# Michaelszeng/GCS-ADMM

Measured on AMD Instinct MI355X. Metric: admm_iterations_per_sec, higher is better.
Workload: dtype f64; 1 GPU; benchmark4; V=42, E=94, n=2, state_dtype=f64, state_columns=incidence, inner_arithmetic=f64, vertex_program=workgroup, vertex_solves=warm start from the previous iteration's record (csrc/warm_start.h), parallelism=1 GPU

## Files before the change

### gcs_admm_amd/csrc/vertex_wg.h

```cpp
#pragma once
#include <type_traits>

#include "gcs_math.h"
#include "step_args.h"
#include "warm_start.h"

#if defined(__HIP_DEVICE_COMPILE__)
#define WG_DEVICE 1
#else
#define WG_DEVICE 0
#endif

namespace gcs_wg {

using gcs_math::REG_DELTA;
using gcs_math::rcp;
using gcs_math::rcp1;
using gcs_math::rsqrt_nr;
using gcs_math::sqrt_nr;

#ifndef GCS_WG_THREADS
#define GCS_WG_THREADS 256
#endif
constexpr int WG_THREADS = GCS_WG_THREADS;
// ... 15 lines not shown
__device__ __forceinline__ int wg_tid()
{
    int t = (int)threadIdx.x;
    asm volatile("" : "+v"(t));
    return t;
}
#define WG_FOR(i, cnt) for (int i = gcs_wg::wg_tid(), i##_end = (cnt); i < i##_end; i += gcs_wg::WG_THREADS)
#define WG_FOR_AT(i, cnt, start) for (int i = (gcs_wg::wg_tid() - (start)) & (gcs_wg::WG_THREADS - 1), i##_end = (cnt); i < i##_end; i += gcs_wg::WG_THREADS)
#define WG_SYNC() gcs_wg::wg_barrier<WG_VM>()
#define WG_ONE() if (gcs_wg::wg_tid() == 0)
#define WG_CONE() if (gcs_wg::wg_tid() == gcs_wg::WG_THREADS - 1)
#define WG_CONE2(l) for (int l = gcs_wg::wg_tid() - (gcs_wg::WG_THREADS - 2); l >= 0 && l < 2; l = 2)
#define WG_WAVE0() if (gcs_wg::wg_tid() < 64)
#define WG_FIRST_WAVES(w, cnt) for (int w = gcs_wg::wg_tid() >> 6; w < (cnt); w += gcs_wg::WG_WAVES)
#define WG_ITEM_FOR(q, i, count, PER)                                                                                          \
    for (int t_ = gcs_wg::wg_tid(), w_ = t_ >> 6, l_ = t_ & 63,                                                                \
             n_ = w_ < gcs_wg::WG_ITEM_WAVES ? (((count) - w_ + gcs_wg::WG_ITEM_WAVES - 1) / gcs_wg::WG_ITEM_WAVES) * (PER) : 0;  \
         l_ < n_; l_ += 64)                                                                                                    \
        if (const int qq_ = l_ / (PER), i = l_ - qq_ * (PER), q = w_ + gcs_wg::WG_ITEM_WAVES * qq_; true)
#define WG_REPL_FOR(i, cnt) for (int i = (gcs_wg::wg_tid() >> 6) < gcs_wg::WG_ITEM_WAVES ? (gcs_wg::wg_tid() & 63) : (cnt), i##_end = (cnt); i < i##_end; i += 64)
#define WG_WAVE_SYNC() gcs_wg::wg_wave_sync<WG_VM>()
#define WG_FENCE() asm volatile("" ::: "memory")
#else
#define WG_FENCE() do { } while (0)
#ifdef GCS_WG_REVERSE
#define WG_FOR(i, cnt) for (int i = (cnt) - 1; i >= 0; --i)
#else
#define WG_FOR(i, cnt) for (int i = 0, i##_end = (cnt); i < i##_end; ++i)
#endif
#define WG_FOR_AT(i, cnt, start) WG_FOR(i, ((void)(start), (cnt)))
#define WG_SYNC() do { } while (0)
#define WG_ONE() if (true)
#define WG_CONE() if (true)
#define WG_CONE2(l) for (int l = 0; l < 2; ++l)
#define WG_WAVE0() if (true)
#define WG_FIRST_WAVES(w, cnt) for (int w = 0; w < (cnt); ++w)
#define WG_ITEM_FOR(q, i, count, PER) WG_FOR(t_, (count) * (PER)) if (const int q = t_ / (PER), i = t_ - q * (PER); true)
#define WG_REPL_FOR(i, cnt) WG_FOR(i, cnt)
#define WG_WAVE_SYNC() do { } while (0)
#endif

#if defined(GCS_WG_TIMING) && defined(__HIPCC__)
__device__ unsigned long long g_wg_cycles[64];
__device__ unsigned long long g_wg_counts[64];
__device__ unsigned long long g_wg_wave_cycles[64 * 8];
#endif
#if defined(GCS_WG_TIMING) && WG_DEVICE
__device__ __forceinline__ void wg_stamp(int id, unsigned long long &last)
{
    if (blockIdx.x == 0) {
        const unsigned long long t = __builtin_amdgcn_s_memtime();
        if (threadIdx.x == 0) {
            atomicAdd(&g_wg_cycles[id], t - last);
            atomicAdd(&g_wg_counts[id], 1ull);
        }
        last = t;
    }
}
__device__ __forceinline__ void wg_arrive(int id, unsigned long long last)
{
    if (blockIdx.x == 0) {
        const unsigned long long t = __builtin_amdgcn_s_memtime();
        if ((threadIdx.x & 63) == 0) atomicAdd(&g_wg_wave_cycles[id * 8 + ((threadIdx.x >> 6) & 7)], t - last);
    }
}
#define WG_ARRIVE(id) gcs_wg::wg_arrive(id, wg_last_stamp)
#define WG_STAMP(id) gcs_wg::wg_stamp(id, wg_last_stamp)
#define WG_STAMP_INIT() unsigned long long wg_last_stamp = __builtin_amdgcn_s_memtime()
#else
#define WG_STAMP(id) do { } while (0)
#define WG_ARRIVE(id) do { } while (0)
#define WG_STAMP_INIT() do { } while (0)
#endif

struct Place {
    int off = 0;
    GCS_HD int at(int cnt)
    {
        const int start = off & (WG_THREADS - 1);
        off = (off + cnt + 63) & ~63;
        return start;
    }
};

template <int N> struct WD {
    static constexpr int NW = 2 * N + 1, NX = 2 * N, NB1 = 4 * N + 1, Q = N + 1, NS = N * (N + 1) / 2;
    static constexpr int TA = 2 * NS + 2 * N + 1;
};

constexpr int pad2(int x) { return (x + 1) & ~1; }
template <int N> struct WSoc {
    static constexpr int Q = N + 1;
    static constexpr int SS = 0, LS = Q, WB = 2 * Q, LT = 3 * Q, CV = LT + Q, SU = CV + N, DSSA = SU + N * N, DLSA = DSSA + Q,
                         DSS = DLSA + Q, DLS = DSS + Q, KS = DLS + Q, SIZE = KS + Q;
};
enum { SC_T = 0, SC_DT, SC_DTA, SC_ALPHA, SC_CONEFAIL, SC_C0, SC_ETA, SC_GT, SC_AMAXC, SC_C1C, SC_C2C, SC_AMAXC2, SC_N = 12 };
template <int N> struct WL {
    using D = WD<N>;
    static constexpr int NW = D::NW, NX = D::NX, NB1 = D::NB1;
    static constexpr int CEN = 0, XV = CEN + pad2(N), DX = XV + pad2(NX), NU = DX + pad2(NX), DNU = NU + pad2(2 * NW),
                         BS = DNU + pad2(2 * NW), BSI = BS + pad2(2 * NW * NW), BXS = BSI + pad2(2 * NW * NW),
                         PIVS = BXS + pad2(2 * NW * NX), BG = PIVS + pad2(2 * NW), XBG = BG + pad2(2 * NW), XBX = XBG + pad2(2 * NX),
                         XS = XBX + pad2(2 * NX * NX), RP = XS + pad2(NX * N), VV = RP + pad2(2 * NW), WW = VV + pad2(2 * NW), M = WW + pad2(2 * NW),
                         PIVM = M + pad2(NB1 * NB1), RHS = PIVM + pad2(NB1), SOL = RHS + pad2(NB1),
                         SOC = SOL + pad2(NB1), PQ = SOC + pad2(WSoc<N>::SIZE), PC = PQ + pad2(NX + NW), SC = PC + pad2(NX + NW), RED = SC + pad2(SC_N), FIXED = RED + 3 * 3 * WG_WAVES;
    static constexpr int P = 0, DW = P + pad2(NW), TG = DW + pad2(NW), TF = TG + pad2(NW), LB = TF + pad2(N), KB = LB + 2, DLB = KB + 2,
                         PIV = DLB + 2, G0 = PIV + pad2(NW), GU = G0 + pad2(NW), GX = GU + pad2(NW), TE = GX + pad2(NX),
                         RV = TE + pad2(NW), K = RV + pad2(NW), X = K + pad2(NW * NW), B = X + pad2(NW * NX), ROWS = B + pad2(NW * NW);
    static GCS_HD int unit_stride(int m) { return (ROWS + 12 * m) | 1; }
    static GCS_HD int total(int U, int m) { return FIXED + pad2(U * unit_stride(m)) + pad2(m * N) + pad2(m); }
    static GCS_HD int units_doubles(int U, int m) { return pad2(U * unit_stride(m)); }
};
template <int N> struct WLBox {
    using G = WL<N>;
    using D = WD<N>;
    static constexpr int NW = D::NW, NX = D::NX, NB1 = D::NB1;
    static constexpr int CEN = G::CEN, XV = G::XV, DX = G::DX, NU = G::NU, DNU = G::DNU, BS = G::BS, BSI = G::BSI, BXS = G::BXS, PIVS = G::PIVS,
                         BG = G::BG, XBG = G::XBG, XBX = G::XBX, XS = G::XS, RP = G::RP, VV = G::VV, WW = G::WW, M = G::M, PIVM = G::PIVM,
                         RHS = G::RHS, SOL = G::SOL, SOC = G::SOC, PQ = G::PQ, PC = G::PC, SC = G::SC, RED = G::RED, FIXED = G::FIXED;
    static constexpr int P = G::P, DW = G::DW, TG = G::TG, TF = G::TF, LB = G::LB, KB = G::KB, DLB = G::DLB, G0 = G::G0, GU = G::GU, GX = G::GX,
                         TE = G::TE, RV = G::RV;
    static constexpr int KD = G::K, KY = KD + pad2(NX), KYY = KY + pad2(NX), XD = KYY + 2, XY = XD + pad2(NX),
                         BD = XY + pad2(NX), BW = BD + pad2(NX), BRS = BW + pad2(NW), BQ = BRS + 2, ROWS = BQ + pad2(NX);
    static GCS_HD int unit_stride(int m) { return (ROWS + 12 * m) | 1; }
    static GCS_HD int total(int U, int m) { return FIXED + pad2(U * unit_stride(m)) + pad2(m * N) + pad2(m); }
    static GCS_HD int units_doubles(int U, int m) { return pad2(U * unit_stride(m)); }
};
template <int N> GCS_HD int wg_lds_doubles(int U, int m, bool box = false) { return box ? WLBox<N>::total(U, m) : WL<N>::total(U, m); }
constexpr int WG_MAX_N = 8;
inline bool wg_has_box(int n) { return n == 3 || n == 6; }
inline int wg_lds_doubles_n(int n, int U, int m, bool box = false)
{
    box = box && wg_has_box(n);
    switch (n) {
    case 1: return wg_lds_doubles<1>(U, m);
    case 2: return wg_lds_doubles<2>(U, m);
    case 3: return wg_lds_doubles<3>(U, m, box);
    case 4: return wg_lds_doubles<4>(U, m);
    case 5: return wg_lds_doubles<5>(U, m);
    case 6: return wg_lds_doubles<6>(U, m, box);
    case 7: return wg_lds_doubles<7>(U, m);
    default: return wg_lds_doubles<8>(U, m);
    }
}

struct alignas(8) WgF2 { float a, b; };

template <class T> struct WgArgs : gcsadmm_k::StepArgs<T> {
    int n_vtx;
    const int *vtx;
    const double *prox_q = nullptr, *prox_c = nullptr;
    const int *order = nullptr;
    int *unit_iters = nullptr;
};

struct Red3 { double mn, s1, s2; };

#if WG_DEVICE
template <int SH> __device__ __forceinline__ double dpp_row_shr(double x, double ident)
{
    const int ilo = __double2loint(ident), ihi = __double2hiint(ident);
    const int lo = __builtin_amdgcn_update_dpp(ilo, __double2loint(x), 0x110 + SH, 0xf, 0xf, false);
    const int hi = __builtin_amdgcn_update_dpp(ihi, __double2hiint(x), 0x110 + SH, 0xf, 0xf, false);
    return __hiloint2double(hi, lo);
}
__device__ __forceinline__ double lane_bcast(double x, int lane)
// ... 142 lines not shown
#pragma unroll
        for (int k = i + 1; k < DIM; ++k) s -= Lm[k * DIM + i] * x[k];
        x[i] = s;
        if constexpr (LOWREG) out[i * ldo + c] = s;
        if constexpr (DIM > 9) WG_FENCE();
    }
    if constexpr (!LOWREG) {
#pragma unroll
        for (int i = 0; i < DIM; ++i) out[i * ldo + c] = x[i];
    }
}

template <int Q> GCS_HD void soc_apply_W(const double *wb, double eta, const double *x, double *y)
{
    double dd = 0;
#pragma unroll
    for (int k = 1; k < Q; ++k) dd += wb[k] * x[k];
    const double f = x[0] + dd * rcp(1.0 + wb[0]);
    y[0] = eta * (wb[0] * x[0] + dd);
#pragma unroll
    for (int k = 1; k < Q; ++k) y[k] = eta * (x[k] + wb[k] * f);
}
template <int Q> GCS_HD void soc_apply_Wi(const double *wb, double eta, const double *x, double *y)
{
    double dd = 0;
#pragma unroll
    for (int k = 1; k < Q; ++k) dd += wb[k] * x[k];
    const double ieta = rcp(eta), f = -x[0] + dd * rcp(1.0 + wb[0]);
    y[0] = ieta * (wb[0] * x[0] - dd);
#pragma unroll
    for (int k = 1; k < Q; ++k) y[k] = ieta * (x[k] + wb[k] * f);
}
template <int Q> GCS_HD void soc_apply_W2(const double *wb, double eta, const double *x, double *y)
{
    double vx = wb[0] * x[0];
#pragma unroll
    for (int k = 1; k < Q; ++k) vx -= wb[k] * x[k];
    const double ieta = rcp(eta), ie2 = ieta * ieta;
    y[0] = ie2 * (2.0 * wb[0] * vx - x[0]);
#pragma unroll
    for (int k = 1; k < Q; ++k) y[k] = ie2 * (x[k] - 2.0 * wb[k] * vx);
}

#define WG_ROWS_BEGIN_(pl, DS)                                                                                                 \
    WG_FOR_AT(rt_, (BOX ? U * 2 * N : U * m2), (pl).at(BOX ? U * 2 * N : U * m2)) {                                            \
        int u, i, jk_;                                                                                                         \
        if constexpr (BOX) { u = rt_ / (2 * N); const int ik_ = rt_ - u * (2 * N); i = ik_ / N; jk_ = ik_ - i * N; }           \
        else { u = fdiv(rt_, inv_m2); const int rem_ = rt_ - u * m2; i = rem_ >= m; jk_ = rem_ - i * m; }                      \
        double *un = UN(u);                                                                                                    \
        double ap_ = 0, ax_ = 0, adp_ = 0, adx_ = 0;                                                                           \
        if constexpr (BOX) {                                                                                                   \
            ap_ = un[W::P + i * N + jk_]; ax_ = sm[W::XV + i * N + jk_];                                                       \
            if (DS) { adp_ = un[W::DW + i * N + jk_]; adx_ = sm[W::DX + i * N + jk_]; }                                        \
        } else {                                                                                                               \
            _Pragma("unroll") for (int k_ = 0; k_ < N; ++k_) {                                                                 \
                const double a_ = A[jk_ * N + k_];                                                                             \
                ap_ += a_ * un[W::P + i * N + k_]; ax_ += a_ * sm[W::XV + i * N + k_];                                         \
                if (DS) { adp_ += a_ * un[W::DW + i * N + k_]; adx_ += a_ * sm[W::DX + i * N + k_]; }                          \
            }                                                                                                                  \
        }                                                                                                                      \
        const double yy_ = un[W::P + 2 * N], dy_ = DS ? un[W::DW + 2 * N] : 0.0;                                               \
        _Pragma("unroll") for (int rq_ = 0; rq_ < (BOX ? 4 : 2); ++rq_) {                                                      \
            const int ty = BOX ? rq_ >> 1 : rq_, j = BOX ? jk_ + (rq_ & 1) * N : jk_, ro = ty * m2 + i * m + j;                \
            const double sg_ = (BOX && (rq_ & 1)) ? -1.0 : 1.0, b_ = BC[j];                                                    \
            const double s = ty == 0 ? b_ * yy_ - sg_ * ap_ : b_ * (1.0 - yy_) - sg_ * (ax_ - ap_);                            \
            const double ds = ty == 0 ? b_ * dy_ - sg_ * adp_ : -(b_ * dy_) - sg_ * (adx_ - adp_);                             \
            (void)ds;
#define WG_ROWS_BEGIN(pl) WG_ROWS_BEGIN_(pl, false)
#define WG_ROWS_BEGIN_DS(pl) WG_ROWS_BEGIN_(pl, true)
#define WG_ROWS_END() }}

template <int N, class T, bool BOX = false, bool SPLIT = false>
GCS_HD void wg_solve_vertex(const WgArgs<T> &a, int v, double rho, double mu_scale, double *sm, int &status_out, int &iters_out,
                            double *units = nullptr)
{
    using D = WD<N>;
    using SO = WSoc<N>;
    using W = std::conditional_t<BOX, WLBox<N>, WL<N>>;
    constexpr int NW = D::NW, NX = D::NX, NB1 = D::NB1, Q = D::Q, NS = D::NS, TA = D::TA;
#ifndef GCS_WG_CONE_PAIR_MAXN
#define GCS_WG_CONE_PAIR_MAXN 3
#endif
    constexpr bool CONE_PAIR = N <= GCS_WG_CONE_PAIR_MAXN;
    const bool prox = a.prox_q != nullptr;
    const int lo = a.inc_ptr[v], d = prox ? 0 : a.inc_ptr[v + 1] - lo, d_in = prox ? 0 : a.deg_in[v], d_out = d - d_in;
    const bool sides = d > 0;
    const int p0 = a.poly_ptr[v], m = a.poly_ptr[v + 1] - p0;
    const int U = d + 1, R = 4 * m, m2 = 2 * m;
    const int US = W::unit_stride(m);
    const float inv_m2 = 1.0f / (float)m2;
    double *const UB = SPLIT ? units : sm + W::FIXED;
    auto UN = [&](int u) -> double * { return UB + u * US; };
    constexpr bool WG_VM = SPLIT;
    const int oLAM = W::ROWS, oR1 = W::ROWS + R, oR2 = W::ROWS + 2 * R;
    double *const PA = sm + W::FIXED + (SPLIT ? 0 : pad2(U * US));
    const double *A = PA, *BC = PA + pad2(m * N), *CEN = sm + W::CEN;
    double *SOC = sm + W::SOC, *SC = sm + W::SC;
    int red_phase = 0;
    WG_STAMP_INIT();
    const int deg = (4 * m + 2) * (d + 1) + 1;
    const double inv_deg = 1.0 / (double)deg;
    auto side_of = [&](int u) { return (u - 1) >= d_in ? 1 : 0; };
    auto side_lo = [&](int s) { return s ? d_in + 1 : 1; };
    auto side_hi = [&](int s) { return s ? d : d_in; };

    using WR = gcs_ws::WRec<N>;
    double *const wrec = (a.warm != nullptr && !prox) ? a.warm + a.warm_ptr[v] : nullptr;
    const int WUS = WR::unit_stride(m);
    double dtm = 0.0;
    Place pl0;
    WG_FOR_AT(t, d * NW, pl0.at(d * NW)) {
        const int e = t / NW, w = t - e * NW, edge = a.inc_edge[lo + e];
        const bool out = e >= d_in;
        const int inc = gcsadmm_k::state_column(a, lo, e, edge, out);
        double *un = UN(e + 1);
        const double Tw = gcsadmm_k::consensus_target(a, w, edge, inc, mu_scale);
        int slot = -1;
        if (w == 2 * N) slot = 2 * N;
        else if (out) slot = w;
        else if (w < N) { un[W::TF + w] = Tw; un[W::TG + N + w] = 0.0; }
        else slot = w - N;
        if (slot >= 0) {
            un[W::TG + slot] = Tw;
            if (wrec) dtm = fmax(dtm, fabs(Tw - wrec[WR::UNITS + (e + 1) * WUS + WR::TG + slot]));
        }
    }
    WG_FOR_AT(t, m * N, pl0.at(m * N)) PA[t] = a.poly_A[(size_t)p0 * N + t];
    WG_FOR_AT(j, m + N, pl0.at(m + N)) {
        if (j < m) PA[pad2(m * N) + j] = a.poly_bc[p0 + j];
        else sm[W::CEN + (j - m)] = a.center[(size_t)v * N + (j - m)];
    }
    if (prox) {
        WG_FOR(k, NX + NW) {
            sm[W::PQ + k] = a.prox_q[(size_t)v * (NX + NW) + k];
            sm[W::PC + k] = a.prox_c[(size_t)v * (NX + NW) + k];
        }
    }
    bool use_warm = false;
    double mu_ref = gcs_ws::WS_COLD_REF, ws_dT = -1.0;
    if (wrec) {
        const Red3 rt = wg_reduce<WG_VM>(Red3{-dtm, 0.0, 0.0}, sm + W::RED, red_phase);
        const bool comparable = wg_uniform((int)(wrec[0] == 1.0 && wrec[1] == rho)) != 0;
        ws_dT = wg_uniform(comparable ? -rt.mn * rho : -1.0);
        use_warm = wg_uniform((int)(comparable && ws_dT <= gcs_ws::ws_theta(wrec))) != 0;
        if (use_warm) mu_ref = wg_uniform(fmax(gcs_ws::WS_MU_MIN, gcs_ws::WS_KAPPA * ws_dT));
    }
    const bool ws_started_warm = use_warm;
    const float inv_R2 = 1.0f / (float)(R / 2);

    WG_STAMP(0);
    auto gval = [&](const double *un, int u, int k, bool wk) {
        double g = un[W::G0 + k];
        if (wk) {
            g += un[W::GU + k];
            if (u == 0 && k < 2 * N) g += k < N ? -SOC[SO::KS + 1 + k] : SOC[SO::KS + 1 + (k - N)];
        }
        return g;
    };
    auto te_tasks = [&](Place &pl, bool wk) {
        WG_FOR_AT(t, d * NW, pl.at(d * NW)) {
            const int u = 1 + t / NW, i = t - (u - 1) * NW;
            double *un = UN(u);
            double s = 0;
            if constexpr (BOX) {
                double wg = 0;
#pragma unroll
                for (int k = 0; k < NW; ++k) wg += un[W::BW + k] * gval(un, u, k, wk);
                s = -(un[W::BRS] * un[W::BW + i]) * wg;
                if (i < 2 * N) s -= un[W::BD + i] * gval(un, u, i, wk);
            } else {
#pragma unroll
                for (int k = 0; k < NW; ++k) s -= un[W::B + i * NW + k] * gval(un, u, k, wk);
            }
            un[W::TE + i] = s;
        }
    };
    auto bg_tasks = [&](Place &pl) {
        WG_FOR_AT(t, 2 * NW, pl.at(2 * NW)) {
            const int s = t / NW, i = t - s * NW;
            double acc = 0;
#pragma unroll 4
            for (int u = side_lo(s); u <= side_hi(s); ++u) acc += UN(u)[W::TE + i];
            sm[W::BG + t] = acc;
        }
        WG_FOR_AT(t, 2 * NX, pl.at(2 * NX)) {
            const int part = t / NX, c = t - part * NX, h = c / N;
            const int ulo = part ? 1 + d / 2 : 1, uhi = part ? d : d / 2;
            double acc = 0;
#pragma unroll 2
            for (int u = ulo; u <= uhi; ++u) {
                const double *un = UN(u);
                if constexpr (BOX) acc += un[W::XD + c] * un[W::TE + c] + un[W::XY + c] * un[W::TE + 2 * N];
                else {
#pragma unroll
                    for (int k = 0; k < N; ++k) acc += un[W::X + (h * N + k) * NX + c] * un[W::TE + h * N + k];
                    acc += un[W::X + 2 * N * NX + c] * un[W::TE + 2 * N];
                }
            }
            sm[W::XBG + t] = acc;
        }
    };
    auto v_tasks = [&](Place &pl) {
        WG_FOR_AT(t, 2 * NW, pl.at(2 * NW)) {
            const int s = t / NW, i = t - s * NW;
            const double *Bsi = sm + W::BSI + s * NW * NW;
            double acc = 0;
#pragma unroll
            for (int k = 0; k < NW; ++k) acc += Bsi[i * NW + k] * (sm[W::RP + s * NW + k] - sm[W::BG + s * NW + k]);
            sm[W::VV + t] = acc;
        }
    };
    auto rhs_tasks = [&](Place &pl, bool wk) {
        const double *u0 = UN(0);
        auto base_z = [&](int i) { return -gval(u0, 0, i, wk) - sm[W::VV + i] - sm[W::VV + NW + i]; };
        WG_FOR_AT(q, NX, pl.at(NX)) {
            double r = -REG_DELTA * sm[W::XV + q] - sm[W::XBG + q] - sm[W::XBG + NX + q];
            if (prox) r -= sm[W::PQ + q] * (sm[W::XV + q] + CEN[q < N ? q : q - N] - sm[W::PC + q]);
            if (wk) r -= sm[W::SOL + q];
            for (int s = 0; s < 2; ++s) {
                const double *BXs = sm + W::BXS + s * NW * NX;
#pragma unroll
                for (int i = 0; i < NW; ++i) r -= BXs[i * NX + q] * sm[W::VV + s * NW + i];
            }
            sm[W::RHS + q] = r;
        }
        WG_FOR_AT(k, N, pl.at(N))
            sm[W::RHS + NX + k] = base_z(k) + SOC[SO::CV + k] * SC[SC_GT] * rcp(SC[SC_C0]);
        WG_FOR_AT(k, N, pl.at(N))
            sm[W::RHS + NX + N + k] = base_z(k) + base_z(N + k);
        WG_FOR_AT(k, 1, pl.at(1)) sm[W::RHS + NX + 2 * N + k] = base_z(2 * N);
    };
    auto solve_head = [&](bool wk) {
        {
            Place pl;
            te_tasks(pl, wk);
            if (wk) {
                WG_FOR_AT(q, NX, pl.at(NX)) {
                    double acc = 0;
#pragma unroll 4
                    for (int u = 0; u <= d; ++u) acc += UN(u)[W::GX + q];
                    sm[W::SOL + q] = acc;
                }
            }
        }
        WG_ARRIVE(30);
        WG_SYNC();
        WG_STAMP(30);
        { Place pl; bg_tasks(pl); }
        WG_ARRIVE(31);
        WG_SYNC();
        WG_STAMP(31);
        { Place pl; v_tasks(pl); }
        WG_ARRIVE(32);
        WG_SYNC();
        WG_STAMP(32);
        { Place pl; rhs_tasks(pl, wk); }
        WG_ARRIVE(33);
        WG_SYNC();
        WG_STAMP(33);
    };
    auto cone_dir = [&](int dt_slot, bool wk, double (&xs)[Q], double (&dl)[Q]) {
        const double *u0 = UN(0);
        double wb[Q], ys[Q];
        xs[0] = SC[dt_slot];
#pragma unroll
        for (int k = 0; k < N; ++k) xs[1 + k] = u0[W::DW + k] - u0[W::DW + N + k];
#pragma unroll
        for (int k = 0; k < Q; ++k) wb[k] = SOC[SO::WB + k];
        soc_apply_W2<Q>(wb, SC[SC_ETA], xs, ys);
#pragma unroll
        for (int k = 0; k < Q; ++k) dl[k] = (wk ? SOC[SO::KS + k] : 0.0) - SOC[SO::LS + k] - ys[k];
    };
    auto solve_tail = [&](int dt_slot, bool wk) {
        WG_WAVE0() wave_ldl_solve<NB1>(sm + W::M, sm + W::PIVM, sm + W::RHS, sm + W::SOL);
        WG_ARRIVE(34);
        WG_SYNC();
        WG_STAMP(34);
        auto dzeta = [&](int i) { return i < N ? sm[W::SOL + NX + i] + sm[W::SOL + NX + N + i] : sm[W::SOL + NX + i]; };
        Place plw;
        WG_FOR_AT(t, 2 * NW, plw.at(2 * NW)) {
            const int s = t / NW, i = t - s * NW;
            const double *BXs = sm + W::BXS + s * NW * NX;
            double acc = dzeta(i) + (sm[W::RP + t] - sm[W::BG + t]);
#pragma unroll
            for (int c = 0; c < NX; ++c) acc += BXs[i * NX + c] * sm[W::SOL + c];
            sm[W::WW + t] = acc;
        }
        WG_FOR_AT(t, NX + NW + 1, plw.at(NX + NW + 1)) {
            if (t < NX) sm[W::DX + t] = sm[W::SOL + t];
            else if (t < NX + NW) UN(0)[W::DW + (t - NX)] = dzeta(t - NX);
            else {
                double acc = -SC[SC_GT];
#pragma unroll
                for (int k = 0; k < N; ++k) acc -= SOC[SO::CV + k] * sm[W::SOL + NX + k];
                SC[dt_slot] = acc * rcp(SC[SC_C0]);
            }
        }
        WG_ARRIVE(36);
        WG_SYNC();
        WG_STAMP(36);
        auto cone_bounds = [&](int l) {
            const int oDS = wk ? SO::DSS : SO::DSSA, oDL = wk ? SO::DLS : SO::DLSA;
            double xs[Q], dl[Q], bs[Q], dr[Q];
            cone_dir(dt_slot, wk, xs, dl);
            double c1c = 0, c2c = 0;
#pragma unroll
            for (int k = 0; k < Q; ++k) {
                const double sk = SOC[SO::SS + k], lk = SOC[SO::LS + k];
                SOC[oDS + k] = xs[k]; SOC[oDL + k] = dl[k];
                c1c += sk * dl[k] + lk * xs[k];
                c2c += xs[k] * dl[k];
                bs[k] = l == 1 ? lk : sk; dr[k] = l == 1 ? dl[k] : xs[k];
            }
            SC[SC_C1C] = c1c; SC[SC_C2C] = c2c;
            SC[l == 1 ? SC_AMAXC2 : SC_AMAXC] = gcs_math::soc_max_step<Q>(bs, dr);
            if (l == 2) SC[SC_AMAXC2] = gcs_math::soc_max_step<Q>(SOC + SO::LS, dl);
        };
        if constexpr (CONE_PAIR) { WG_CONE2(l) cone_bounds(l); }
        else { WG_CONE() cone_bounds(2); }
        WG_REPL_FOR(t, 2 * NW) {
            const int s = t / NW, i = t - s * NW;
            const double *Bsi = sm + W::BSI + s * NW * NW;
            double acc = 0;
#pragma unroll
            for (int k = 0; k < NW; ++k) acc += Bsi[i * NW + k] * sm[W::WW + s * NW + k];
            sm[W::DNU + t] = acc;
        }
        WG_WAVE_SYNC();
        WG_ITEM_FOR(q, i, d, NW) {
            const int u = 1 + q;
            double *un = UN(u);
            double acc = -gval(un, u, i, wk) + sm[W::DNU + side_of(u) * NW + i];
            if constexpr (BOX) {
                if (i < 2 * N) acc -= un[W::XD + i] * sm[W::DX + i];
                else {
#pragma unroll
                    for (int c = 0; c < NX; ++c) acc -= un[W::XY + c] * sm[W::DX + c];
                }
            } else if (i < 2 * N) {
                const int h = i / N;
#pragma unroll
                for (int k = 0; k < N; ++k) acc -= un[W::X + i * NX + h * N + k] * sm[W::DX + h * N + k];
            } else {
#pragma unroll
                for (int c = 0; c < NX; ++c) acc -= un[W::X + i * NX + c] * sm[W::DX + c];
            }
            un[W::RV + i] = acc;
        }
        WG_WAVE_SYNC();
        WG_ITEM_FOR(q, i, d, NW) {
            double *un = UN(1 + q);
            double acc = 0;
            if constexpr (BOX) {
                double wr = 0;
#pragma unroll
                for (int k = 0; k < NW; ++k) wr += un[W::BW + k] * un[W::RV + k];
                acc = (un[W::BRS] * un[W::BW + i]) * wr;
                if (i < 2 * N) acc += un[W::BD + i] * un[W::RV + i];
            } else {
#pragma unroll
                for (int k = 0; k < NW; ++k) acc += un[W::B + i * NW + k] * un[W::RV + k];
            }
            un[W::DW + i] = acc;
        }
        WG_ARRIVE(39);
        WG_SYNC();
        WG_STAMP(39);
    };

    int status = -1, it = 0, it_total = 0, stalled = 0;
    bool saved = false, init_pending = true;
#define WG_FAIL_OR_RESTART()                                                                                                   \
    {                                                                                                                          \
        if (!use_warm) break;                                                                                                  \
        it_total += it; it = -1;                                                                                               \
        use_warm = false; mu_ref = gcs_ws::WS_COLD_REF; init_pending = true;                                                   \
        WG_SYNC();                                                                                                             \
        continue;                                                                                                              \
    }
    for (it = 0;; ++it) {
    if (init_pending) {
        init_pending = false; stalled = 0; saved = false;
        Place pls;
        if (use_warm) {
            const double *wu = wrec + WR::UNITS;
            WG_FOR_AT(t, U * NW, pls.at(U * NW)) {
                const int u = t / NW, k = t - u * NW;
                UN(u)[W::P + k] = wu[u * WUS + WR::P + k];
            }
            WG_FOR_AT(t, U * (R / 2), pls.at(U * (R / 2))) {
                const int u = fdiv(t, inv_R2), r2 = t - u * (R / 2);
                const WgF2 v = reinterpret_cast<const WgF2 *>(wu + u * WUS + WR::LAM)[r2];
                UN(u)[oLAM + 2 * r2] = (double)v.a; UN(u)[oLAM + 2 * r2 + 1] = (double)v.b;
            }
            WG_FOR_AT(t, 2 * U, pls.at(2 * U)) UN(t >> 1)[W::LB + (t & 1)] = wu[(t >> 1) * WUS + WR::LB + (t & 1)];
            WG_FOR_AT(k, NX + 2 * NW, pls.at(NX + 2 * NW)) {
                if (k < NX) sm[W::XV + k] = wrec[WR::XV + k];
                else sm[W::NU + (k - NX)] = wrec[WR::NU + (k - NX)];
            }
        } else {
            WG_FOR_AT(t, U * NW, pls.at(U * NW)) {
                const int u = t / NW, k = t - u * NW;
                double val = 0.0;
                if (k == 2 * N) val = u == 0 ? 0.5 : 0.5 / (double)(side_of(u) ? d_out : d_in);
                UN(u)[W::P + k] = val;
            }
            WG_FOR_AT(k, NX + 2 * NW, pls.at(NX + 2 * NW)) {
                if (k < NX) sm[W::XV + k] = 0.0;
                else sm[W::NU + (k - NX)] = 0.0;
            }
            WG_ONE() {
                SC[SC_T] = 1.0;
                SOC[SO::LS] = 1.0;
                for (int k = 1; k < Q; ++k) SOC[SO::LS + k] = 0.0;
            }
        }
        WG_SYNC();
    }
        const bool first_warm = use_warm && it == 0;
        double acc = 0.0; int bad = 0;
        Place plr;
        WG_ROWS_BEGIN(plr)
            const double is = rcp1(s);
            if (it == 0 && !use_warm) un[oLAM + ro] = is;
            const double l = un[oLAM + ro];
            un[oR1 + ro] = l * is;
            acc += s * l;
            if (!(s > 0.0)) bad = 1;
        WG_ROWS_END()
        WG_FOR_AT(u, U, plr.at(U)) {
// ... 251 lines not shown
            double (&li)[NS] = a;
#pragma unroll
            for (int c = 0; c < N; ++c)
#pragma unroll
                for (int i = c; i < N; ++i) {
                    double sx = (i == c) ? 1.0 : 0.0;
#pragma unroll
                    for (int k = c; k < i; ++k) sx -= a[pki(i, k)] * li[pki(k, c)];
                    li[pki(i, c)] = sx * pv[i];
                }
#pragma unroll
            for (int r = 0; r < N; ++r)
#pragma unroll
                for (int c = 0; c <= r; ++c) {
                    double acc = 0;
#pragma unroll
                    for (int i = r; i < N; ++i) acc += li[pki(i, r)] * li[pki(i, c)];
                    un[W::B + (h * N + r) * NW + h * N + c] = acc;
                    un[W::B + (h * N + c) * NW + h * N + r] = acc;
                }
            double lv[N], ch = 0;
#pragma unroll
            for (int i = 0; i < N; ++i) {
                double acc = 0;
#pragma unroll
                for (int c = 0; c <= i; ++c) acc += li[pki(i, c)] * kv[c];
                lv[i] = acc;
                ch += acc * acc;
            }
#pragma unroll
            for (int r = 0; r < N; ++r) {
                double acc = 0;
#pragma unroll
                for (int i = r; i < N; ++i) acc += li[pki(i, r)] * lv[i];
                un[W::PIV + h * N + r] = acc;
            }
            un[W::RV + h] = ch;
            }
        }
        WG_ARRIVE(3);
        WG_SYNC();
        WG_STAMP(3);
        if constexpr (BOX) {
            WG_FOR(t, d * NW) {
                const int u = 1 + t / NW, c = t - (u - 1) * NW;
                double *un = UN(u);
                if (c < 2 * N) un[W::BQ + c] = un[W::BW + c] * un[W::XD + c] - un[W::XY + c];
                else {
                    const double kap = un[W::KYY];
                    un[W::BRS] = rcp(gcs_math::pivot_floor(kap - un[W::RV] - un[W::RV + 1], kap));
                    un[W::BW + 2 * N] = -1.0;
                }
            }
            WG_ARRIVE(4);
            WG_SYNC();
            WG_STAMP(4);
            if (!first_warm) {
                { Place plx; te_tasks(plx, false); }
                WG_SYNC();
            }
            WG_STAMP(5);
        } else {
        WG_FOR(t, d * NW * NW) {
            const int u = 1 + t / (NW * NW), ij = t - (u - 1) * (NW * NW), i = ij / NW, j = ij - i * NW;
            double *un = UN(u);
            const double kap = un[W::K + 2 * N * NW + 2 * N];
            const double rs = rcp(gcs_math::pivot_floor(kap - un[W::RV] - un[W::RV + 1], kap));
            const double wi = i < 2 * N ? un[W::PIV + i] : -1.0, wj = j < 2 * N ? un[W::PIV + j] : -1.0;
            const double base = (i < 2 * N && j < 2 * N && i / N == j / N) ? un[W::B + ij] : 0.0;
            un[W::B + ij] = base + wi * wj * rs;
        }
        WG_ARRIVE(4);
        WG_SYNC();
        WG_STAMP(4);
        Place plx;
        WG_FOR_AT(t, d * NW * NX, plx.at(d * NW * NX)) {
            const int u = 1 + t / (NW * NX), ic = t - (u - 1) * (NW * NX), i = ic / NX, c = ic - i * NX, h = c / N;
            double *un = UN(u);
            double s = un[W::B + i * NW + 2 * N] * un[W::X + 2 * N * NX + c];
#pragma unroll
            for (int k = 0; k < N; ++k) s += un[W::B + i * NW + h * N + k] * un[W::X + (h * N + k) * NX + c];
            un[W::K + ic] = s;
        }
        if (!first_warm) te_tasks(plx, false);
        WG_ARRIVE(5);
        WG_SYNC();
        WG_STAMP(5);
        }
        Place plq;
        constexpr int NWT = NW * (NW + 1) / 2, NXT = NX * (NX + 1) / 2;
        WG_FOR_AT(t0, 2 * NWT, plq.at(2 * NWT)) {
            const int s = t0 / NWT;
            int i, j;
            tri_decode(t0 - s * NWT, i, j);
            const int q = i * NW + j, t = s * NW * NW + q;
            double acc2 = 0;
            if constexpr (BOX) {
#pragma unroll 4
                for (int u = side_lo(s); u <= side_hi(s); ++u) {
                    const double *un = UN(u);
                    acc2 += (un[W::BRS] * un[W::BW + i]) * un[W::BW + j];
                    if (i == j && i < 2 * N) acc2 += un[W::BD + i];
                }
            } else {
#pragma unroll 4
                for (int u = side_lo(s); u <= side_hi(s); ++u) acc2 += UN(u)[W::B + q];
            }
            sm[W::BS + t] = acc2;
        }
        WG_FOR_AT(tt, 2 * NW * NX, plq.at(2 * NW * NX)) {
            const int s = tt / (NW * NX), q = tt - s * NW * NX;
            double acc2 = 0;
            if constexpr (BOX) {
                const int i = q / NX, c = q - i * NX;
#pragma unroll 4
                for (int u = side_lo(s); u <= side_hi(s); ++u) {
                    const double *un = UN(u);
                    acc2 += (un[W::BRS] * un[W::BW + i]) * un[W::BQ + c];
                    if (i == c) acc2 += un[W::BD + c] * un[W::XD + c];
                }
            } else {
#pragma unroll 4
                for (int u = side_lo(s); u <= side_hi(s); ++u) acc2 += UN(u)[W::K + q];
            }
            sm[W::BXS + tt] = acc2;
        }
        WG_FOR_AT(tp0, 2 * NXT, plq.at(2 * NXT)) {
            const int part = tp0 / NXT;
            int r, c;
            tri_decode(tp0 - part * NXT, r, c);
            const int tp = part * NX * NX + r * NX + c, h = r / N;
            (void)h;
            const int ulo = part ? 1 + d / 2 : 1, uhi = part ? d : d / 2;
            double acc2 = 0;
#pragma unroll 2
            for (int u = ulo; u <= uhi; ++u) {
                const double *un = UN(u);
                if constexpr (BOX) {
                    acc2 += (un[W::BRS] * un[W::BQ + r]) * un[W::BQ + c];
                    if (r == c) acc2 += (un[W::XD + r] * un[W::XD + r]) * un[W::BD + r];
                } else {
#pragma unroll
                    for (int k = 0; k < N; ++k) acc2 += un[W::X + (h * N + k) * NX + r] * un[W::K + (h * N + k) * NX + c];
                    acc2 += un[W::X + 2 * N * NX + r] * un[W::K + 2 * N * NX + c];
                }
            }
            sm[W::XBX + tp] = acc2;
        }
        WG_FOR_AT(tt, NX * N, plq.at(NX * N)) {
            const int r = tt / N, c = (r / N) * N + (tt - r * N);
            double acc2 = 0;
            if constexpr (BOX) {
                if (c == r) {
#pragma unroll 4
                    for (int u = 0; u <= d; ++u) acc2 += UN(u)[W::XD + r];
                }
            } else {
#pragma unroll 4
                for (int u = 0; u <= d; ++u) acc2 += UN(u)[W::X + r * NX + c];
            }
            sm[W::XS + tt] = acc2;
        }
        WG_FOR_AT(tt, 2 * NW, plq.at(2 * NW)) {
            const int s = tt / NW, k = tt - s * NW;
            double acc2 = UN(0)[W::P + k];
#pragma unroll 4
            for (int u = side_lo(s); u <= side_hi(s); ++u) acc2 -= UN(u)[W::P + k];
            sm[W::RP + tt] = acc2;
        }
        if (!first_warm) bg_tasks(plq);
        WG_ARRIVE(6);
        WG_SYNC();
        WG_STAMP(6);
        Place ply;
        if (sides) {
            WG_FIRST_WAVES(sd, 2) wave_ldl<NW>(sm + W::BS + sd * NW * NW, sm + W::PIVS + sd * NW);
            WG_ARRIVE(7);
            WG_SYNC();
            WG_STAMP(7);
            WG_FOR(t, 2 * NW) {
                const int s = t / NW, c = t - s * NW;
                ldl_inverse_col<NW, (!BOX && NW > 9)>(sm + W::BS + s * NW * NW, sm + W::PIVS + s * NW, c, sm + W::BSI + s * NW * NW, NW);
            }
            WG_SYNC();
            WG_FOR_AT(t, 2 * NW * NX, ply.at(2 * NW * NX)) {
                const int s = t / (NW * NX), ic = t - s * NW * NX, i = ic / NX, c = ic - i * NX;
                const double *Bsi = sm + W::BSI + s * NW * NW, *BXs = sm + W::BXS + s * NW * NX;
                double acc2 = 0;
#pragma unroll
                for (int k = 0; k < NW; ++k) acc2 += Bsi[i * NW + k] * BXs[k * NX + c];
                sm[W::BS + s * NW * NW + ic] = acc2;
            }
        } else {
            WG_FOR(t, 2 * NW * NW) { sm[W::BSI + t] = 0.0; sm[W::BS + t] = 0.0; }
            WG_SYNC();
        }
        if (!first_warm) v_tasks(ply);
        WG_ARRIVE(9);
        WG_SYNC();
        WG_STAMP(9);
        {
            const double *YS0 = sm + W::BS, *YS1 = sm + W::BS + NW * NW, *u0 = UN(0);
            auto x0 = [&](int i, int c) {
                if constexpr (BOX) return i == c ? u0[W::XD + c] : (i == 2 * N ? u0[W::XY + c] : 0.0);
                else return u0[W::X + i * NX + c];
            };
            auto k0 = [&](int hi, int lo) {
                if constexpr (BOX) return hi == lo ? (hi < 2 * N ? u0[W::KD + hi] : u0[W::KYY]) : (hi == 2 * N ? u0[W::KY + lo] : 0.0);
                else return u0[W::K + hi * NW + lo];
            };
            auto zx = [&](int i, int c) { return x0(i, c) + YS0[i * NX + c] + YS1[i * NX + c]; };
            auto zz = [&](int i, int k) {
                const int hi = i > k ? i : k, lo = i > k ? k : i;
                return k0(hi, lo) + sm[W::BSI + hi * NW + lo] + sm[W::BSI + NW * NW + hi * NW + lo];
            };
            Place plm;
            WG_FOR_AT(t, NX * (NX + 1) / 2, plm.at(NX * (NX + 1) / 2)) {
                int r, c;
                tri_decode(t, r, c);
                double val = (r == c ? REG_DELTA + (prox ? sm[W::PQ + r] : 0.0) : 0.0) - sm[W::XBX + r * NX + c] - sm[W::XBX + NX * NX + r * NX + c];
                if (r / N == c / N) val -= sm[W::XS + r * N + (c - (c / N) * N)];
#pragma unroll
                for (int k = 0; k < NW; ++k)
                    val += sm[W::BXS + k * NX + r] * YS0[k * NX + c] + sm[W::BXS + NW * NX + k * NX + r] * YS1[k * NX + c];
                sm[W::M + r * NB1 + c] = val;
            }
            WG_FOR_AT(t, NW * NX, plm.at(NW * NX)) {
                const int i = t / NX, c = t - i * NX;
                double val = zx(i, c);
                if (i >= N && i < 2 * N) val += zx(i - N, c);
                sm[W::M + (NX + i) * NB1 + c] = val;
            }
            WG_FOR_AT(t, NW * (NW + 1) / 2, plm.at(NW * (NW + 1) / 2)) {
                int i, k;
                tri_decode(t, i, k);
                const bool rz2 = i >= N && i < 2 * N, cz2 = k >= N && k < 2 * N;
                double val = zz(i, k);
                if (cz2) val += zz(i, k - N);
                if (rz2) val += zz(i - N, k);
                if (rz2 && cz2) val += zz(i - N, k - N);
                if (i < N && k < N) val += SOC[SO::SU + i * N + k];
                sm[W::M + (NX + i) * NB1 + NX + k] = val;
            }
            if (!first_warm) rhs_tasks(plm, false);
        }
        WG_ARRIVE(10);
        WG_SYNC();
        WG_STAMP(10);
        WG_WAVE0() wave_ldl<NB1>(sm + W::M, sm + W::PIVM);
        WG_ARRIVE(11);
        WG_SYNC();
        WG_STAMP(11);
        WG_STAMP(12);
        double rmax = 0.0, c1 = 0.0, c2 = 0.0, amax_cone = 1e300;
        double sigmu;
        if (first_warm) {
            Place plb;
            WG_ROWS_BEGIN(plb)
                un[oR1 + ro] = 0.0;
                un[oR2 + ro] = rcp1(s);
            WG_ROWS_END()
            WG_FOR_AT(u, U, plb.at(U)) { double *un = UN(u); un[W::KB] = 0.0; un[W::KB + 1] = 0.0; }
            sigmu = mu_ref;
            WG_ARRIVE(14);
            WG_SYNC();
            WG_STAMP(14);
        } else {
        solve_tail(SC_DTA, false);
        WG_STAMP(13);
        Place plb;
        WG_ROWS_BEGIN_DS(plb)
            const double l = un[oLAM + ro], is = rcp1(s);
            const double q = ds * is, dl = -l - l * q;
            rmax = fmax(rmax, fmax(-q, 1.0 + q));
            c1 += s * dl + l * ds; c2 += ds * dl;
            un[oR1 + ro] = ds * dl;
            un[oR2 + ro] = is;
        WG_ROWS_END()
        WG_FOR_AT(u, U, plb.at(U)) {
            double *un = UN(u);
            const double yy = un[W::P + 2 * N], dy = un[W::DW + 2 * N];
            const double s5 = yy, s6 = 1.0 - yy, l5 = un[W::LB], l6 = un[W::LB + 1];
            const double q5 = dy * rcp1(s5), q6 = -dy * rcp1(s6);
            const double dl5 = -l5 - l5 * q5, dl6 = -l6 - l6 * q6;
            rmax = fmax(rmax, fmax(fmax(-q5, 1.0 + q5), fmax(-q6, 1.0 + q6)));
            c1 += s5 * dl5 + l5 * dy + s6 * dl6 - l6 * dy; c2 += dy * dl5 - dy * dl6;
            un[W::KB] = dy * dl5; un[W::KB + 1] = -dy * dl6;
        }
        WG_CONE() { amax_cone = fmin(SC[SC_AMAXC], SC[SC_AMAXC2]); c1 += SC[SC_C1C]; c2 += SC[SC_C2C]; }
        WG_ARRIVE(14);
        const Red3 rb = wg_reduce<WG_VM>(Red3{fmin(rmax > 0.0 ? rcp1(rmax) : 1e300, amax_cone), c1, c2}, sm + W::RED, red_phase);
        WG_STAMP(14);
        {
            const double al = fmin(1.0, rb.mn);
            const double mu_aff = (gap + al * rb.s1 + al * al * rb.s2) * inv_deg;
            sigmu = wg_uniform(gcs_math::centring(mu_aff * rcp(mu)) * mu);
        }
        }
        WG_CONE() {
            double wb[Q], a1[Q], a2[Q], pr[Q], qv[Q], xs[Q], lt[Q], ss[Q];
            const double eta = SC[SC_ETA];
#pragma unroll
            for (int k = 0; k < Q; ++k) { wb[k] = SOC[SO::WB + k]; xs[k] = SOC[SO::DSSA + k]; lt[k] = SOC[SO::LT + k]; ss[k] = SOC[SO::SS + k]; }
            soc_apply_Wi<Q>(wb, eta, xs, a1);
#pragma unroll
            for (int k = 0; k < Q; ++k) xs[k] = SOC[SO::DLSA + k];
            soc_apply_W<Q>(wb, eta, xs, a2);
            double dsum = 0;
#pragma unroll
            for (int k = 0; k < Q; ++k) dsum += a1[k] * a2[k];
            pr[0] = dsum;
#pragma unroll
            for (int k = 1; k < Q; ++k) pr[k] = a1[0] * a2[k] + a2[0] * a1[k];
            const double det = gcs_math::soc_det<Q>(lt);
            double ld1 = 0;
#pragma unroll
            for (int k = 1; k < Q; ++k) ld1 += lt[k] * pr[k];
            qv[0] = (lt[0] * pr[0] - ld1) * rcp(det);
            const double ilt0 = rcp(lt[0]);
#pragma unroll
            for (int k = 1; k < Q; ++k) qv[k] = (pr[k] - qv[0] * lt[k]) * ilt0;
            const double smd = sigmu * rcp(gcs_math::soc_det<Q>(ss));
            soc_apply_Wi<Q>(wb, eta, qv, a1);
#pragma unroll
            for (int i = 0; i < Q; ++i) SOC[SO::KS + i] = smd * (i == 0 ? ss[0] : -ss[i]) - (first_warm ? 0.0 : a1[i]);
            SC[SC_GT] = 1.0 - SOC[SO::KS];
        }
// ... 139 lines not shown
```

Before: 9936 iterations/s.

## Fuse vertex solve head stages for N=2 to cut workgroup barriers

For N=2 (non-box), the solve head now uses two barrier-separated phases instead of four. It computes BG/XBG directly from per-unit B/K data, and it folds the V-vector products into the RHS via BSI and Y (BS) matrices. The tail also drops a barrier by recomputing dnu rows inline, and the cone direction now comes from the solution vector. This trades extra redundant arithmetic and shared-memory reads per thread for fewer workgroup synchronisations per solve.

New measurement: 9249 iterations/s. 0.931x the previous value.

```diff
diff --git a/gcs_admm_amd/csrc/vertex_wg.h b/gcs_admm_amd/csrc/vertex_wg.h
--- a/gcs_admm_amd/csrc/vertex_wg.h
+++ b/gcs_admm_amd/csrc/vertex_wg.h
@@ -121,6 +121,12 @@
         return start;
     }
 };
+
+#ifdef GCS_WG_FUSED_SOLVE
+constexpr bool wg_fused_solve(int n) { return n == 2 && (GCS_WG_FUSED_SOLVE) != 0; }
+#else
+constexpr bool wg_fused_solve(int n) { return n == 2; }
+#endif
 
 template <int N> struct WD {
     static constexpr int NW = 2 * N + 1, NX = 2 * N, NB1 = 4 * N + 1, Q = N + 1, NS = N * (N + 1) / 2;
@@ -429,6 +435,7 @@
 #define GCS_WG_CONE_PAIR_MAXN 3
 #endif
     constexpr bool CONE_PAIR = N <= GCS_WG_CONE_PAIR_MAXN;
+    constexpr bool FUSED = !BOX && wg_fused_solve(N);
     const bool prox = a.prox_q != nullptr;
     const int lo = a.inc_ptr[v], d = prox ? 0 : a.inc_ptr[v + 1] - lo, d_in = prox ? 0 : a.deg_in[v], d_out = d - d_in;
     const bool sides = d > 0;
@@ -559,15 +566,36 @@
     };
     auto rhs_tasks = [&](Place &pl, bool wk) {
         const double *u0 = UN(0);
-        auto base_z = [&](int i) { return -gval(u0, 0, i, wk) - sm[W::VV + i] - sm[W::VV + NW + i]; };
+        auto rb = [&](int s, int k) { return sm[W::RP + s * NW + k] - sm[W::BG + s * NW + k]; };
+        auto base_z = [&](int i) {
+            if constexpr (FUSED) {
+                double v0 = 0, v1 = 0;
+#pragma unroll
+                for (int k = 0; k < NW; ++k) {
+                    v0 += sm[W::BSI + i * NW + k] * rb(0, k);
+                    v1 += sm[W::BSI + NW * NW + i * NW + k] * rb(1, k);
+                }
+                return -gval(u0, 0, i, wk) - (v0 + v1);
+            } else return -gval(u0, 0, i, wk) - sm[W::VV + i] - sm[W::VV + NW + i];
+        };
         WG_FOR_AT(q, NX, pl.at(NX)) {
             double r = -REG_DELTA * sm[W::XV + q] - sm[W::XBG + q] - sm[W::XBG + NX + q];
             if (prox) r -= sm[W::PQ + q] * (sm[W::XV + q] + CEN[q < N ? q : q - N] - sm[W::PC + q]);
             if (wk) r -= sm[W::SOL + q];
+            if constexpr (FUSED) {
+                double y0 = 0, y1 = 0;
+#pragma unroll
+                for (int i = 0; i < NW; ++i) {
+                    y0 += sm[W::BS + i * NX + q] * rb(0, i);
+                    y1 += sm[W::BS + NW * NW + i * NX + q] * rb(1, i);
+                }
+                r -= y0 + y1;
+            } else {
             for (int s = 0; s < 2; ++s) {
                 const double *BXs = sm + W::BXS + s * NW * NX;
 #pragma unroll
                 for (int i = 0; i < NW; ++i) r -= BXs[i * NX + q] * sm[W::VV + s * NW + i];
+            }
             }
             sm[W::RHS + q] = r;
         }
@@ -577,7 +605,75 @@
             sm[W::RHS + NX + N + k] = base_z(k) + base_z(N + k);
         WG_FOR_AT(k, 1, pl.at(1)) sm[W::RHS + NX + 2 * N + k] = base_z(2 * N);
     };
+    auto gx_tasks = [&](Place &pl) {
+        WG_FOR_AT(q, NX, pl.at(NX)) {
+            double acc = 0;
+#pragma unroll 4
+            for (int u = 0; u <= d; ++u) acc += UN(u)[W::GX + q];
+            sm[W::SOL + q] = acc;
+        }
+    };
+    auto head1_tasks = [&](Place &pl, bool wk) {
+        te_tasks(pl, wk);
+        if constexpr (FUSED) {
+            WG_FOR_AT(t, 2 * NW, pl.at(2 * NW)) {
+                const int s = t / NW, i = t - s * NW, hi = side_hi(s);
+                double a0 = 0, a1 = 0;
+                int u = side_lo(s);
+                for (; u < hi; u += 2) {
+                    const double *p = UN(u), *q = UN(u + 1);
+#pragma unroll
+                    for (int k = 0; k < NW; ++k) {
+                        a0 -= p[W::B + i * NW + k] * gval(p, u, k, wk);
+                        a1 -= q[W::B + i * NW + k] * gval(q, u + 1, k, wk);
+                    }
+                }
+                if (u == hi) {
+                    const double *p = UN(u);
+#pragma unroll
+                    for (int k = 0; k < NW; ++k) a0 -= p[W::B + i * NW + k] * gval(p, u, k, wk);
+                }
+                sm[W::BG + t] = a0 + a1;
+            }
+            WG_FOR_AT(t, 2 * NX, pl.at(2 * NX)) {
+                const int part = t / NX, c = t - part * NX;
+                const int hi = part ? d : d / 2;
+                double a0 = 0, a1 = 0;
+                int u = part ? 1 + d / 2 : 1;
+                for (; u < hi; u += 2) {
+                    const double *p = UN(u), *q = UN(u + 1);
+#pragma unroll
+                    for (int k = 0; k < NW; ++k) {
+                        a0 -= p[W::K + k * NX + c] * gval(p, u, k, wk);
+                        a1 -= q[W::K + k * NX + c] * gval(q, u + 1, k, wk);
+                    }
+                }
+                if (u == hi) {
+                    const double *p = UN(u);
+#pragma unroll
+                    for (int k = 0; k < NW; ++k) a0 -= p[W::K + k * NX + c] * gval(p, u, k, wk);
+                }
+                sm[W::XBG + t] = a0 + a1;
+            }
+        }
+        if (wk) gx_tasks(pl);
+    };
+    auto head2_tasks = [&](Place &pl, bool wk) {
+        rhs_tasks(pl, wk);
+        v_tasks(pl);
+    };
     auto solve_head = [&](bool wk) {
+        if constexpr (FUSED) {
+            { Place pl; head1_tasks(pl, wk); }
+            WG_ARRIVE(30);
+            WG_SYNC();
+            WG_STAMP(30);
+            { Place pl; head2_tasks(pl, wk); }
+            WG_ARRIVE(33);
+            WG_SYNC();
+            WG_STAMP(33);
+            return;
+        }
         {
             Place pl;
             te_tasks(pl, wk);
@@ -609,9 +705,16 @@
     auto cone_dir = [&](int dt_slot, bool wk, double (&xs)[Q], double (&dl)[Q]) {
         const double *u0 = UN(0);
         double wb[Q], ys[Q];
+        if constexpr (FUSED) {
+            double acc = -SC[SC_GT];
+#pragma unroll
+            for (int k = 0; k < N; ++k) { xs[1 + k] = sm[W::SOL + NX + k]; acc -= SOC[SO::CV + k] * xs[1 + k]; }
+            xs[0] = acc * rcp(SC[SC_C0]);
+        } else {
         xs[0] = SC[dt_slot];
 #pragma unroll
         for (int k = 0; k < N; ++k) xs[1 + k] = u0[W::DW + k] - u0[W::DW + N + k];
+        }
 #pragma unroll
         for (int k = 0; k < Q; ++k) wb[k] = SOC[SO::WB + k];
         soc_apply_W2<Q>(wb, SC[SC_ETA], xs, ys);
@@ -624,7 +727,21 @@
         WG_SYNC();
         WG_STAMP(34);
         auto dzeta = [&](int i) { return i < N ? sm[W::SOL + NX + i] + sm[W::SOL + NX + N + i] : sm[W::SOL + NX + i]; };
+        auto dnu_row = [&](int s, int i) {
+            const double *Bsi = sm + W::BSI + s * NW * NW, *Ys = sm + W::BS + s * NW * NW;
+            double a0 = sm[W::VV + s * NW + i], a1 = 0;
+#pragma unroll
+            for (int k = 0; k < NW; ++k) a0 += Bsi[i * NW + k] * dzeta(k);
+#pragma unroll
+            for (int c = 0; c < NX; ++c) a1 += Ys[i * NX + c] * sm[W::SOL + c];
+            return a0 + a1;
+        };
         Place plw;
+        if constexpr (FUSED) {
+            plw.off = (WG_ITEM_WAVES - 1) * 64;
+            WG_FOR_AT(t, 2 * NW, plw.at(2 * NW)) sm[W::DNU + t] = dnu_row(t / NW, t - (t / NW) * NW);
+            plw.off = (WG_ITEM_WAVES - 1) * 64 + 2 * NW;
+        } else {
         WG_FOR_AT(t, 2 * NW, plw.at(2 * NW)) {
             const int s = t / NW, i = t - s * NW;
             const double *BXs = sm + W::BXS + s * NW * NX;
@@ -632,6 +749,7 @@
 #pragma unroll
             for (int c = 0; c < NX; ++c) acc += BXs[i * NX + c] * sm[W::SOL + c];
             sm[W::WW + t] = acc;
+        }
         }
         WG_FOR_AT(t, NX + NW + 1, plw.at(NX + NW + 1)) {
             if (t < NX) sm[W::DX + t] = sm[W::SOL + t];
@@ -643,9 +761,11 @@
                 SC[dt_slot] = acc * rcp(SC[SC_C0]);
             }
         }
+        if constexpr (!FUSED) {
         WG_ARRIVE(36);
         WG_SYNC();
         WG_STAMP(36);
+        }
         auto cone_bounds = [&](int l) {
             const int oDS = wk ? SO::DSS : SO::DSSA, oDL = wk ? SO::DLS : SO::DLSA;
             double xs[Q], dl[Q], bs[Q], dr[Q];
@@ -665,6 +785,22 @@
         };
         if constexpr (CONE_PAIR) { WG_CONE2(l) cone_bounds(l); }
         else { WG_CONE() cone_bounds(2); }
+        if constexpr (FUSED) {
+            WG_ITEM_FOR(q, i, d, NW) {
+                const int u = 1 + q;
+                double *un = UN(u);
+                double acc = -gval(un, u, i, wk) + dnu_row(side_of(u), i), ax = 0;
+                if (i < 2 * N) {
+                    const int h = i / N;
+#pragma unroll
+                    for (int k = 0; k < N; ++k) ax += un[W::X + i * NX + h * N + k] * sm[W::SOL + h * N + k];
+                } else {
+#pragma unroll
+                    for (int c = 0; c < NX; ++c) ax += un[W::X + i * NX + c] * sm[W::SOL + c];
+                }
+                un[W::RV + i] = acc - ax;
+            }
+        } else {
         WG_REPL_FOR(t, 2 * NW) {
             const int s = t / NW, i = t - s * NW;
             const double *Bsi = sm + W::BSI + s * NW * NW;
@@ -693,6 +829,7 @@
                 for (int c = 0; c < NX; ++c) acc -= un[W::X + i * NX + c] * sm[W::DX + c];
             }
             un[W::RV + i] = acc;
+        }
         }
         WG_WAVE_SYNC();
         WG_ITEM_FOR(q, i, d, NW) {
@@ -1110,7 +1247,7 @@
             for (int k = 0; k < N; ++k) s += un[W::B + i * NW + h * N + k] * un[W::X + (h * N + k) * NX + c];
             un[W::K + ic] = s;
         }
-        if (!first_warm) te_tasks(plx, false);
+        if constexpr (!FUSED) { if (!first_warm) te_tasks(plx, false); }
         WG_ARRIVE(5);
         WG_SYNC();
         WG_STAMP(5);
@@ -1196,7 +1333,9 @@
             for (int u = side_lo(s); u <= side_hi(s); ++u) acc2 -= UN(u)[W::P + k];
             sm[W::RP + tt] = acc2;
         }
-        if (!first_warm) bg_tasks(plq);
+        if (!first_warm) {
+            if constexpr (FUSED) head1_tasks(plq, false); else bg_tasks(plq);
+        }
         WG_ARRIVE(6);
         WG_SYNC();
         WG_STAMP(6);
@@ -1223,7 +1362,7 @@
             WG_FOR(t, 2 * NW * NW) { sm[W::BSI + t] = 0.0; sm[W::BS + t] = 0.0; }
             WG_SYNC();
         }
-        if (!first_warm) v_tasks(ply);
+        if constexpr (!FUSED) { if (!first_warm) v_tasks(ply); }
         WG_ARRIVE(9);
         WG_SYNC();
         WG_STAMP(9);
@@ -1270,7 +1409,9 @@
                 if (i < N && k < N) val += SOC[SO::SU + i * N + k];
                 sm[W::M + (NX + i) * NB1 + NX + k] = val;
             }
-            if (!first_warm) rhs_tasks(plm, false);
+            if (!first_warm) {
+                if constexpr (FUSED) head2_tasks(plm, false); else rhs_tasks(plm, false);
+            }
         }
         WG_ARRIVE(10);
         WG_SYNC();
```
